# pacificclimate/VIC

Hardware: AMD Instinct MI355X
Metric: cell-timesteps/s (higher is better)
Workload: dtype f64

## Files before the change

vic_amd/csrc/vic_hru_io.hpp:

```cpp
#pragma once
#include <cstddef>
#include "vic_step.hpp"

using namespace vic;

struct LaunchMap {
  int nslot = 0, ccount = 0;
  __host__ __device__ int nblocks(int gcount) const {
    if (nslot == 0) return (gcount + 63) / 64;
    const int ncb = (ccount + 63) / 64;
    return (ncb + 7) / 8 * 8 * nslot;
  }
  VIC_DEV int index(int block, int lane, int gcount) const {
    if (nslot == 0) { const int gi = block * 64 + lane; return gi < gcount ? gi : -1; }
    const int q = block >> 3, cb = q / nslot * 8 + (block & 7), cell = cb * 64 + lane;
    return cell < ccount ? (q % nslot) * ccount + cell : -1;
  }
};

struct KArgs {
  Opt o;
  LaunchMap map;
  int ncell, nhru, nveg_rows, write_fluxes;
  const double* veglib;
  const double* cell_params;
  const int* hpi;
  const double* hpd;
  const double* forcing;
  const unsigned char* snowflag;
  const int* fcol;
  int ncol;
  Dmy dmy;
  double* sd;
  int* si;
  double* flux;
  int* hru_err;
  const int* glist;
  int gcount;
  unsigned long long* ctx;
  double* pin;
  double* ts;
  double* pout;
  int* pslot;
  int* hstate;
  int* list;
  int* count;
  int list_cap;
  int* hkey;
  double* pimp;
  int* lastexp;
  int* jl;
  int phase;
  const int* valid;
};

template <int NN>
VIC_DEV void load_state(const KArgs& a, int g, HruWork<NN>& w, bool node_props = true) {
  const int Nn = a.o.Nnode;
  const size_t nh = a.nhru;
  const double* __restrict__ sd = a.sd;
  const int* __restrict__ si = a.si;
#define SD(row) sd[(size_t)(row) * nh + g]
#define SI(row) si[(size_t)(row) * nh + g]
#pragma unroll
  for (int l = 0; l < 3; l++) { w.moist[l] = SD(SD_MOIST0 + l); w.ice[l] = SD(SD_ICE0 + l); w.layer_T[l] = SD(SD_LAYER_T0 + l); w.evap[l] = 0; }
  SoilEnergy& so = w.so; SnowEnergy& se = w.se; Snow& s = w.snow;
  so.snow_flux = SD(SD_SNOW_FLUX); so.grnd_flux = SD(SD_GRND_FLUX); so.deltaH = SD(SD_DELTAH); so.fusion = SD(SD_FUSION);
  so.LongUnderOut = SD(SD_LONGUNDEROUT); se.Tfoliage = SD(SD_TFOLIAGE);
  s.albedo = SD(SD_SNOW_ALBEDO); s.coldcontent = SD(SD_SNOW_COLDCONTENT); s.coverage = SD(SD_SNOW_COVERAGE);
  s.density = SD(SD_SNOW_DENSITY); s.depth = SD(SD_SNOW_DEPTH); s.pack_temp = SD(SD_SNOW_PACK_TEMP);
  s.pack_water = SD(SD_SNOW_PACK_WATER); s.snow_canopy = SD(SD_SNOW_CANOPY); s.surf_temp = SD(SD_SNOW_SURF_TEMP);
  s.surf_water = SD(SD_SNOW_SURF_WATER); s.swq = SD(SD_SNOW_SWQ); s.tmp_int_storage = SD(SD_SNOW_TMP_INT_STORAGE);
  s.store_swq = SD(SD_SNOW_STORE_SWQ); s.store_coverage = SD(SD_SNOW_STORE_COVERAGE); s.swq_slope = SD(SD_SNOW_SWQ_SLOPE);
  s.max_swq = SD(SD_SNOW_MAX_SWQ);
  s.blowing_flux = 0; s.canopy_vapor_flux = 0; s.mass_error = 0; s.melt = 0; s.Qnet = 0; s.surface_flux = 0; s.vapor_flux = 0;
  w.vv.Wdew = SD(SD_WDEW); w.vv.canopyevap = 0; w.vv.throughfall = 0;
  w.Tcanopy = SD(SD_TCANOPY); so.Tsurf = SD(SD_TSURF); se.AlbedoOver = SD(SD_ALBEDO_OVER); so.AlbedoUnder = SD(SD_ALBEDO_UNDER);
  se.canopy_advection = SD(SD_CANOPY_ADVECTION); se.canopy_latent = SD(SD_CANOPY_LATENT);
  se.canopy_latent_sub = SD(SD_CANOPY_LATENT_SUB); se.canopy_sensible = SD(SD_CANOPY_SENSIBLE);
  se.canopy_refreeze = SD(SD_CANOPY_REFREEZE);
// ... 217 lines not shown
```

vic_amd/csrc/vic_kernels.hpp:

```cpp
#pragma once
#include <cstddef>
#include "vic_glacier.hpp"
#include "vic_profile.hpp"
#include "vic_implicit.hpp"
#include "vic_ctx.hpp"
#include "vic_hru_io.hpp"

using namespace vic;

template <int NN, bool GLAC>
VIC_DEV int hru_prologue(const KArgs& a, int g, const HruId& id, const CellView& cv, const VegLib& vl, const Forcing& fc, const Soil3& s3,
                         HruWork<NN>& w, StepConst& C, bool node_props = true) {
  const Opt& o = a.o;
  const size_t nh = a.nhru;
  const int month = a.dmy.month;
  const int veg_idx = id.veg_idx;
  int err = 0;
  C.veg_idx = veg_idx; C.band = id.band; C.is_art_bare = id.is_art_bare ? 1 : 0;
#pragma unroll
  for (int l = 0; l < 3; l++) C.root[l] = (double)(float)a.hpd[(size_t)(HPD_ROOT0 + l) * nh + g];
  if (o.BLOWING) {
    C.sigma_slope = (double)(float)a.hpd[(size_t)HPD_SIGMA_SLOPE * nh + g]; C.lag_one = (double)(float)a.hpd[(size_t)HPD_LAG_ONE * nh + g];
    C.fetch = (double)(float)a.hpd[(size_t)HPD_FETCH * nh + g];
  } else { C.sigma_slope = 0; C.lag_one = 0; C.fetch = 0; }
// ... 115 lines not shown
      const double blow[4] = {C.sigma_slope, C.lag_one, C.fetch, (double)C.is_art_bare};
      ok = surface_fluxes_glac<NN>(o, cv, vl, s3, fc, a.dmy, C.veg_idx, C.band, C.bare_albedo, C.aero_pet, C.Ra, C.U, C.zref, C.z0, C.disp, blow, w, w.gl,
                                   w.so.NetLongUnder, ge, nlu, nsu, sui);
      SoilEnergy& so = w.so; SnowEnergy& se = w.se;
      so.snow_flux = ge.snow_flux; so.grnd_flux = ge.grnd_flux; so.deltaH = 0; so.fusion = 0; so.LongUnderOut = ge.LongUnderOut;
      so.AlbedoUnder = ge.AlbedoUnder; so.advected_sensible = ge.advected_sensible; so.advection = ge.advection;
      so.deltaCC = ge.deltaCC; so.refreeze_energy = ge.refreeze_energy; so.error = ge.error; so.latent = ge.latent;
      so.latent_sub = ge.latent_sub; so.sensible = ge.sensible; so.NetLongUnder = nlu; so.NetShortUnder = nsu; so.NetShortGrnd = 0;
      se.canopy_advection = 0; se.canopy_latent = 0; se.canopy_latent_sub = 0; se.canopy_sensible = 0; se.canopy_refreeze = 0;
      w.AlbedoOver_avg = 0; w.LongOverIn_avg = 0; w.NetLongOver_avg = 0; w.NetShortOver_avg = 0; w.ShortOverIn_avg = 0;
      w.ShortUnderIn_avg = sui;
      w.deltaCC_glac = ge.deltaCC_glac; w.glacier_flux = ge.glacier_flux; w.glacier_melt_energy = ge.glacier_melt_energy;
      if (!isnan(w.gl.cum_mass_balance) && !isnan(w.gl.mass_balance)) w.gl.cum_mass_balance += w.gl.mass_balance;
    } else {
      ok = surface_fluxes<NN>(o, cv, vl, s3, fc, a.dmy, C, w);
    }
    if (!ok) err |= VICGPU_CELLERR_SOLVER;
  }
  hru_epilogue<NN>(a, g, cv, s3, C, w, err, GLAC);
  PROF_ADD(0, t_kernel);
  PROF_WAVE(0);
  PROF_LANE(1);
}

template <int NN, bool FIRST, bool MULTI>
__global__ __launch_bounds__(64) VIC_WAVES_PER_EU(1, 1) void vic_fd_stage(const KArgs a) {
  const int gi = a.map.index(blockIdx.x, threadIdx.x, a.gcount);
  if (gi < 0) return;
  const int g = a.glist ? a.glist[gi] : gi;
  const Opt& o = a.o;
  const HruId id = hru_id(a, g);
  if (id.run && id.is_glacier) return;
  if (FIRST && a.valid && a.valid[id.c] != CELL_VALID) { a.hstate[g] = 0; return; }
  if (FIRST && !id.run) { store_zero_record(a, g); a.hstate[g] = 0; return; }
  if (!FIRST && (a.hstate[g] & HS_STATE) != 2) return;
  CellView cv{a.cell_params, a.ncell, id.c, o.Nnode, o.Nband};
  VegLib vl{a.veglib};
  Forcing fc{a.forcing, a.snowflag, a.ncell, id.c, o.NR + 1, a.fcol[g], a.ncol};
  const Soil3 s3 = load_soil3(cv);
  const int Nn = node_count<NN>(o.Nnode);
  const CtxRef cx = CtxRef::at(a.ctx, ctx_words<NN>(), g);
  HruWork<NN> w;
  StepConst C;
  SubLoop L;
  int err = 0;
  bool more;
  PROF_T0(t_stage);
  if constexpr (FIRST) {
    err = hru_prologue<NN, false>(a, g, id, cv, vl, fc, s3, w, C, false);
    PROF_ADD(1, t_stage);
    more = !(err & VICGPU_CELLERR_AERO);
    if (more) sf_begin<NN>(o, fc, C, w, L);
  } else {
    SubStep P;
    SurfEB eb;
    SurfSolve sv;
    ctx_get_words(cx, CO_SV, sv, (int)CW_SV_ITER, (int)CW_SV);
    ctx_get(cx, CO_EBM, static_cast<SurfEBMut&>(eb));
    ctx_get_words(cx, CO_EBC, static_cast<SurfEBConst&>(eb), 0, EBC_W_POST);
    surf_cell_fill(eb, cv, vl, s3, fc, eb.hidx, id.veg_idx, a.dmy.month);
    ctx_get(cx, CO_P, P);
    ctx_get_words(cx, CO_L, L, 0, (int)CW_L_HEAD);
    if (MULTI && L.N_steps > 0) ctx_get_words(cx, CO_L, L, (int)CW_L_HEAD, (int)CW_L);
    else zero_substep_sums(L);
    load_untouched_state<NN>(a, g, w);
    if constexpr (MULTI) {
      ctx_get(cx, CO_C, C);
// ... 77 lines not shown
          }
        if constexpr (NN >= NBUCKET / 2) nfrozen = (nfrozen < NBUCKET / 2 - 1) ? nfrozen : NBUCKET / 2 - 1;
        key = nfrozen + (kink ? NBUCKET / 2 : 0);
        a.hkey[g] = key;
      }
      profile_item_store<NN>(o, cv, s3, w.nd, eb.delta_t, eb.frozen_on != 0, a.pin + (size_t)g * Nn * PREC);
      if (o.IMPLICIT) {
        double* __restrict__ im = a.pimp + (size_t)g * Nn * PIMP;
#pragma unroll
        for (int n = 0; n < NN; n++)
          if (n < Nn) {
            im[n * PIMP + PI_MOIST] = w.nd.moist[n]; im[n * PIMP + PI_ICE] = (n == 0) ? eb.delta_t : w.nd.ice[n];
            im[n * PIMP + PI_KAPPA] = w.nd.kappa[n]; im[n * PIMP + PI_CS] = w.nd.Cs[n];
          }
        a.lastexp[g] = -1;
      }
      a.ts[g] = sv.x;
      a.pslot[g] = 0;
      if (o.QUICK_SOLVE) {
        int tmpNnodes = 0;
#pragma unroll
        for (int n = NN - 1; n >= 0; n--)
          if (n <= Nn - 5 && w.nd.T[n] >= 0 && w.nd.T[(n + 1 < NN) ? n + 1 : n] < 0) tmpNnodes = n + 1;
        if (tmpNnodes == 0) tmpNnodes = (w.nd.T[0] <= 0 && w.nd.T[1] >= 0) ? Nn : 3;
        else tmpNnodes += 4;
        a.jl[g] = (sv.stage == SurfSolve::ROOT_QUICK) ? tmpNnodes - 1 : (o.NOFLUX ? Nn : Nn - 1);
      }
      a.pout[(size_t)g * pout_hru_stride(Nn) + pout_key(Nn, 0)] = NAN;
      a.pout[(size_t)g * pout_hru_stride(Nn) + pout_key(Nn, 1)] = NAN;
      a.hstate[g] = 1 | (cls << HS_CLS_SHIFT);
      pend = true;
      PROF_ADD(14, t_put);
    }
  } else {
    PROF_T0(t_end);
    if (more && !sf_end<NN>(o, cv, s3, C, w, L)) err |= VICGPU_CELLERR_SOLVER;
    PROF_ADD(15, t_end);
    hru_epilogue<NN>(a, g, cv, s3, C, w, err, false);
    a.hstate[g] = 0;
  }
  list_append(a.list, a.count, a.list_cap, pend, key, g);
  PROF_ADD(0, t_stage);
  PROF_WAVE(0);
  PROF_LANE(1);
}

struct EArgs {
  Opt o;
  LaunchMap map;
  int ncell, nhru, Nn;
  const int* glist;
  int gcount;
  const double* cell_params;
  const int* hpi;
  unsigned long long* ctx;
  size_t ctx_words;
  double* pout;
  int* pslot;
  double* ts;
  int* jl;
  int* hstate;
  int* list_next;
  int* count_next;
  int list_cap;
  const int* hkey;
  int* profile_next;
  int* pend_list_next;
  int* pend_count_next;
  int pend_cap;
  int list_thr;
  const int* pend_list_cur;
  const int* pend_prefix;
  const int* npend_cur;
  int implicit;
  const double* veglib;
  const double* forcing;
  const int* fcol;
// ... 114 lines not shown
```

vic_amd/csrc/vic_pipeline.hpp:

```cpp
#pragma once
#include <hip/hip_runtime.h>
#include <stdio.h>
#include <stdlib.h>
#include <string.h>
#include <algorithm>
#include <chrono>
#include <condition_variable>
#include <memory>
#include <mutex>
#include <string>
#include <vector>
#include "vicgpu.h"
#include "vic_profile.hpp"
#include "vic_putdata.hpp"
#include "vic_host.hpp"
#include "vic_implicit.hpp"
#include "vic_ctx.hpp"
#include "vic_hru_io.hpp"
#include "vic_kernels.hpp"
#include "vic_aux_kernels.hpp"
#include "vic_records.hpp"
#include "vic_copy_cells.hpp"
#include "vic_params.hpp"
#include "vic_state_update.hpp"
#include "vic_mix_cells.hpp"

using namespace vic;

#define HIPIGN(call) do { hipError_t ign_ = (call); (void)ign_; } while (0)
#define HIPCHK(ctx, call)                                                                              \
  do {                                                                                                 \
    hipError_t e_ = (call);                                                                            \
    if (e_ != hipSuccess) {                                                                            \
      (ctx)->err = std::string(#call) + ": " + hipGetErrorString(e_);                                  \
      return VICGPU_ERR_HIP;                                                                           \
    }                                                                                                  \
  } while (0)

constexpr int RB_LAG = 3, RB_DEPTH = RB_LAG + 1;
struct FdChunk {
  int c0 = 0, ccount = 0;
  DevBuf<int> d_glist;
  int gcount = 0;
  LaunchMap map;
  DevBuf<int> d_list[2];
  DevBuf<int> d_fb_list, d_fb_count;
  DevBuf<int> d_count;
  DevBuf<int> d_plist[2];
  int list_cap = 0;
  int pend_cap = 0;
  PinnedBuf<int> h_count;
  Stream stream;
  Event done, readback[RB_DEPTH];
  std::string err;
  int status = 0;
  long long rounds = 0, steps = 0;
};

struct Domain {
  int ncell = 0, nhru = 0;
  bool domain_ready = false;
  bool any_glacier = false;
  DevBuf<double> d_cp, d_hpd, d_sd, d_flux, d_cell_out, d_accum;
  DevBuf<int> d_hpi, d_si, d_cell_off, d_cell_list, d_hru_err, d_cell_err;
  DevBuf<int> d_valid;
  bool valid_live = false;
  int ncol = 0;
  std::vector<int> cell_col;
  DevBuf<int> d_cell_col;
  DevBuf<int> d_hru_fcol;
  std::vector<int> cell_off, cell_list, copy_key;
  std::vector<int> cell_class;
  MixPlan mix_plan;
  bool fd = false;
  DevBuf<unsigned long long> d_ctx;
  DevBuf<double> d_pin, d_ts, d_pout;
  DevBuf<int> d_hstate, d_pslot, d_hkey, d_lastexp, d_jl;
  DevBuf<double> d_pimp;
  std::vector<FdChunk> chunks;
  bool put_on = false;
  int out_nrow = 0;
  OutLayout out_lay;
  DevBuf<double> d_out_data, d_out_agg, d_pb;
  DevBuf<unsigned char> d_rowagg;
};

constexpr int COPY_NKEY = 4;
constexpr int COPY_KEY_ROWS[COPY_NKEY] = {HPI_BAND, HPI_VEG_CLASS, HPI_IS_GLACIER, HPI_IS_ARTIFICIAL_BARE};

struct Tuning {
  bool node_newton = false;
  int eval_list_pct = 75;
  int nchunk = 1;
  int profile_waves_pct = 100;
  bool xcd_map = true;
  bool trace_rounds = false;
  bool trace = false;
  bool stats = false;
  int copy_stage_mb = 256;
};
static Tuning read_tuning(int node_solver, int ncell) {
  Tuning t;
  t.node_newton = node_solver == VIC_NODE_SOLVER_NEWTON;
  if (const char* ev = getenv("VICGPU_NODE_SOLVER")) t.node_newton = (strcmp(ev, "newton") == 0);
  if (const char* ev = getenv("VICGPU_EVAL_LIST_PCT")) {
    const int pct = atoi(ev);
    if (pct >= 0 && pct <= 100) t.eval_list_pct = pct;
  }
  t.nchunk = (ncell >= 20000) ? 2 : 1;
  if (const char* ev = getenv("VICGPU_CHUNKS")) t.nchunk = atoi(ev);
  if (t.nchunk < 1) t.nchunk = 1;
  if (t.nchunk > 16) t.nchunk = 16;
  if (t.nchunk > ncell) t.nchunk = ncell;
  t.profile_waves_pct = t.nchunk > 1 ? 50 : 100;
  if (const char* ev = getenv("VICGPU_PROFILE_WAVES_PCT")) {
    const int pct = atoi(ev);
    if (pct >= 5 && pct <= 100) t.profile_waves_pct = pct;
  }
  t.xcd_map = getenv("VICGPU_NO_XCD_MAP") == nullptr;
  t.trace_rounds = getenv("VICGPU_TRACE_ROUNDS") != nullptr;
  t.trace = getenv("VICGPU_TRACE") != nullptr;
  t.stats = getenv("VICGPU_STATS") != nullptr;
  if (const char* ev = getenv("VICGPU_COPY_STAGE_MB")) {
    const int mb = atoi(ev);
    if (mb >= 0 && mb <= 65536) t.copy_stage_mb = mb;
  }
  return t;
}


struct RecordsJoin {
  std::mutex m;
  std::condition_variable cv;
  std::vector<int> arrived;
  int queued = 0;
  int status = 0;
  std::string err;
  void start(int nrecords) { arrived.assign(nrecords, 0); queued = 0; status = 0; err.clear(); }
  bool arrive(int k, int nlane) { std::lock_guard<std::mutex> lk(m); return ++arrived[k] == nlane; }
  void join_queued(int k) { { std::lock_guard<std::mutex> lk(m); queued = k + 1; } cv.notify_all(); }
  int wait_queued(int k, std::string* why) {
    std::unique_lock<std::mutex> lk(m);
    cv.wait(lk, [&]() { return queued > k || status != 0; });
    if (status != 0) *why = err;
    return status;
  }
  void fail(int st, const std::string& why) {
    { std::lock_guard<std::mutex> lk(m); if (status == 0) { status = st; err = why; } }
    cv.notify_all();
  }
};

struct Records {
  int nrow = 0, depth = 0;
  DevBuf<int> d_sel_pos;
// ... 46 lines not shown
    std::vector<int> dmy;
    int nsteps = 0;
    Event uploaded;
    Event released;
    bool upload_pending = false, was_current = false;
    Event derive_t0, derive_t1;
    bool derive_timed = false;
  } slot[2];
  int cur = -1, staged = -1;
  Stream stream, copy_stream;
  Records rec;
  std::vector<Event> ev;
  int ev_used = 0;
  int write_fluxes = 1;
  int steps_done = 0;
  int profile_waves = 0;
  int ev_steps = 0;
  int out_step_ratio = 1;
  int retire_mask = 0;
};

struct PertLists {
  int nsrc;
  const int* col_src;
  int src_base;
  int ngroup;
  const int* col_group;
  int group_base;
  const double* pert;
};

static int* valid_table(const vicgpu_ctx* c) { return c->dom.valid_live ? c->dom.d_valid.get() : nullptr; }

static hipStream_t records_stream(const vicgpu_ctx* c) { return c->rec.dl ? (hipStream_t)c->rec.dl : (hipStream_t)c->stream; }

static void records_report_reduce(vicgpu_ctx* c) {
  Records& R = c->rec;
  float ms = 0;
  if (R.reduce_timed && hipEventElapsedTime(&ms, R.reduce_t0, R.reduce_t1) == hipSuccess)
    fprintf(stderr, "[vicgpu] records reduce: %d groups, %d members, a %s per group, %d rows: %.4f ms\n", R.ngroup, R.nnz,
            R.lane_per_group ? "lane" : "wave", R.nrow, ms);
  R.reduce_timed = false;
}

static void free_records(vicgpu_ctx* c) {
  if (c->rec.depth > 0) HIPIGN(hipStreamSynchronize(records_stream(c)));
  records_report_reduce(c);
  c->rec = Records();
}

static void drop_forcing(vicgpu_ctx* c) {
  c->chunk_steps = 0;
  c->dmy.clear();
  c->cur = c->staged = -1;
  c->d_forcing = nullptr; c->d_snowflag = nullptr;
}

static void free_domain(vicgpu_ctx* c) {
  free_records(c);
  c->dom = Domain();
  drop_forcing(c);
}

static const int* forcing_col_row(const Domain& d) { return d.d_hru_fcol ? d.d_hru_fcol.get() : d.d_hpi.get() + (size_t)HPI_CELL * d.nhru; }

template <int NN>
static hipError_t launch_hru(const KArgs& ka, hipStream_t st, bool ordinary, bool glacier) {
  const int nblk = ka.map.nblocks(ka.gcount);
  if constexpr (NN == 3) {
    if (ordinary) hipLaunchKernelGGL((vic_hru_step<NN, false>), dim3(nblk), dim3(64), 0, st, ka);
  }
  if (glacier) hipLaunchKernelGGL((vic_hru_step<NN, true>), dim3(nblk), dim3(64), 0, st, ka);
  return hipGetLastError();
}

template <int NN>
static hipError_t launch_fd_stage(const KArgs& ka, bool multi, hipStream_t st) {
  const dim3 grid(ka.map.nblocks(ka.gcount)), block(64);
  if (ka.phase == 0) {
    if (multi) hipLaunchKernelGGL((vic_fd_stage<NN, true, true>), grid, block, 0, st, ka);
    else hipLaunchKernelGGL((vic_fd_stage<NN, true, false>), grid, block, 0, st, ka);
  } else {
    if (multi) hipLaunchKernelGGL((vic_fd_stage<NN, false, true>), grid, block, 0, st, ka);
    else hipLaunchKernelGGL((vic_fd_stage<NN, false, false>), grid, block, 0, st, ka);
  }
  return hipGetLastError();
}

using ProfileKernel = void (*)(const PArgs);
template <int NN>
constexpr ProfileKernel profile_kernel(bool newton) {
  if constexpr (NN == 10) return newton ? vic_profile_solve_reg<NN, true> : vic_profile_solve_reg<NN, false>;
  else return newton ? vic_profile_solve_lockstep<NN, true> : vic_profile_solve_lockstep<NN, false>;
}

template <int NN>
static hipError_t launch_profile(const PArgs& pa, int nmax, int resident_waves, bool newton, hipStream_t st) {
  int nblk = (nmax + 63) / 64;
  if (nblk > resident_waves) nblk = resident_waves;
  if (nblk < 1) nblk = 1;
  hipLaunchKernelGGL(profile_kernel<NN>(newton), dim3(nblk), dim3(64), 0, st, pa);
  return hipGetLastError();
}

template <int NN>
static int profile_resident_waves(int device, bool newton) {
  int per_cu = 0, ncu = 0;
  const hipError_t e = hipOccupancyMaxActiveBlocksPerMultiprocessor(&per_cu, profile_kernel<NN>(newton), 64, 0);
  if (e != hipSuccess || per_cu <= 0) per_cu = 8;
  if (hipDeviceGetAttribute(&ncu, hipDeviceAttributeMultiprocessorCount, device) != hipSuccess || ncu <= 0) ncu = 256;
  return per_cu * ncu;
}

constexpr int CNT_LIST_STRIDE = 64, CNT_CURSOR = 128, CNT_NPEND = 160, CNT_PREFIX = 192, CNT_STRIPES = 288,
              CNT_STRIPES_STRIDE = PEND_STRIPES * PEND_CNT_STRIDE, CNT_TOTAL = CNT_STRIPES + 2 * CNT_STRIPES_STRIDE;
static_assert(NBUCKET <= CNT_LIST_STRIDE && CNT_PREFIX + PEND_STRIPES + 1 <= CNT_STRIPES && CNT_STRIPES % 32 == 0, "counter block layout");
static inline int* cnt_list(int* d_count, int l) { return d_count + l * CNT_LIST_STRIDE; }
static inline int* cnt_stripes(int* d_count, int l) { return d_count + CNT_STRIPES + l * CNT_STRIPES_STRIDE; }
static inline int cnt_pending(const int* h_count, int l) {
  int n = 0;
  for (int s = 0; s < PEND_STRIPES; s++) n += h_count[CNT_STRIPES + l * CNT_STRIPES_STRIDE + s * PEND_CNT_STRIDE];
  return n;
}

static int fd_read_count(FdChunk* ch, int which, int* nsolve, int* npending) {
  HIPCHK(ch, hipMemcpyAsync(ch->h_count, ch->d_count, sizeof(int) * CNT_TOTAL, hipMemcpyDeviceToHost, ch->stream));
  HIPCHK(ch, hipStreamSynchronize(ch->stream));
  int n = 0;
  for (int b = 0; b < NBUCKET; b++) n += ch->h_count[which * CNT_LIST_STRIDE + b];
  *nsolve = n;
  *npending = cnt_pending(ch->h_count, which);
  return VICGPU_OK;
}

#define NODE_DISPATCH(Nnode, F, ...)                                                                                          \
  (node_bound(Nnode) == 10 ? F<10>(__VA_ARGS__)                                                                           \
                           : node_bound(Nnode) == VIC_MID_NODES ? F<VIC_MID_NODES>(__VA_ARGS__) : F<VIC_MAX_NODES>(__VA_ARGS__))

static KArgs make_kargs(const vicgpu_ctx* c) {
  const Domain& d = c->dom;
  KArgs ka{};
  ka.o = c->o; ka.ncell = d.ncell; ka.nhru = d.nhru; ka.gcount = d.nhru; ka.nveg_rows = c->nveg_rows;
  ka.write_fluxes = (c->write_fluxes || d.put_on) ? 1 : 0;
  ka.veglib = c->d_veglib; ka.cell_params = d.d_cp; ka.hpi = d.d_hpi; ka.hpd = d.d_hpd; ka.sd = d.d_sd; ka.si = d.d_si; ka.flux = d.d_flux;
  ka.hru_err = d.d_hru_err; ka.ctx = d.d_ctx; ka.pin = d.d_pin; ka.ts = d.d_ts; ka.pout = d.d_pout; ka.pslot = d.d_pslot;
  ka.hstate = d.d_hstate; ka.hkey = d.d_hkey; ka.pimp = d.d_pimp; ka.lastexp = d.d_lastexp; ka.jl = d.d_jl;
  ka.valid = valid_table(c);
  ka.fcol = forcing_col_row(d); ka.ncol = d.ncol;
// ... 8 lines not shown
  ca.valid = valid_table(c); ca.retire_mask = c->retire_mask;
  return ca;
}
static PArgs profile_args(const vicgpu_ctx* c, const FdChunk* ch) {
  const Domain& d = c->dom;
  PArgs pa{};
  pa.pin = d.d_pin; pa.ts = d.d_ts; pa.pout = d.d_pout; pa.pslot = d.d_pslot; pa.jl = d.d_jl; pa.cap = ch->list_cap;
  pa.Nn = c->o.Nnode; pa.NOFLUX = c->o.NOFLUX; pa.EXP_TRANS = c->o.EXP_TRANS; pa.TFALLBACK = c->o.TFALLBACK;
  pa.next = ch->d_count + CNT_CURSOR; pa.pend_prefix = ch->d_count + CNT_PREFIX; pa.pend_out = ch->d_count + CNT_NPEND;
  return pa;
}
static EArgs eval_args(const vicgpu_ctx* c, const FdChunk* ch, const KArgs& ka) {
  const Domain& d = c->dom;
  EArgs ea{};
  ea.o = c->o; ea.ncell = d.ncell; ea.nhru = d.nhru; ea.Nn = c->o.Nnode; ea.glist = ch->d_glist; ea.gcount = ch->gcount; ea.map = ch->map;
  ea.cell_params = d.d_cp; ea.hpi = d.d_hpi; ea.ctx = d.d_ctx; ea.ctx_words = NODE_DISPATCH(c->o.Nnode, ctx_words);
  ea.pout = d.d_pout; ea.pslot = d.d_pslot; ea.ts = d.d_ts; ea.jl = d.d_jl; ea.hstate = d.d_hstate; ea.hkey = d.d_hkey;
  ea.list_cap = ch->list_cap; ea.pend_cap = ch->pend_cap; ea.profile_next = ch->d_count + CNT_CURSOR;
  ea.pend_prefix = ch->d_count + CNT_PREFIX; ea.npend_cur = ch->d_count + CNT_NPEND; ea.implicit = c->o.IMPLICIT;
  ea.veglib = c->d_veglib; ea.forcing = ka.forcing; ea.fcol = ka.fcol; ea.ncol = ka.ncol; ea.month = ka.dmy.month;
  return ea;
}
static IArgs implicit_args(const vicgpu_ctx* c, const FdChunk* ch) {
  const Domain& d = c->dom;
  IArgs ia{};
  ia.ncell = d.ncell; ia.nhru = d.nhru; ia.Nband = c->o.Nband; ia.pimp = d.d_pimp; ia.hpi = d.d_hpi; ia.cell_params = d.d_cp;
  ia.hkey = d.d_hkey; ia.lastexp = d.d_lastexp; ia.fb_list = ch->d_fb_list; ia.fb_count = ch->d_fb_count; ia.cursor = ch->d_fb_count + NBUCKET;
  return ia;
}

static int fd_step(vicgpu_ctx* c, FdChunk* ch, KArgs ka) {
  const int Nn = c->o.Nnode;
  hipStream_t st = ch->stream;
  if (c->dom.any_glacier) HIPCHK(ch, NODE_DISPATCH(Nn, launch_hru, ka, st, false, true));
  HIPCHK(ch, hipMemsetAsync(ch->d_count, 0, sizeof(int) * CNT_TOTAL, st));
  int cur = 0;
  ka.phase = 0; ka.list = ch->d_list[cur]; ka.count = cnt_list(ch->d_count, cur); ka.list_cap = ch->list_cap;
  HIPCHK(ch, NODE_DISPATCH(Nn, launch_fd_stage, ka, c->o.NF > 1, st));
  PArgs pa = profile_args(c, ch);
  EArgs ea = eval_args(c, ch, ka);
  const IArgs ia = c->o.IMPLICIT ? implicit_args(c, ch) : IArgs{};
  const int list_thr = (int)((long long)ch->gcount * c->tune.eval_list_pct / 100);
  const int FREE_ROUNDS = 6;
  const int nsub = c->o.NF;
  for (int p = 1; p <= nsub; p++) {
    int nmax = ch->gcount;
    int npend = -1;
    int rb_list[RB_DEPTH];
    int rb_first = -1;
    for (int round = 0;; round++) {
      pa.list = ch->d_list[cur]; pa.count = cnt_list(ch->d_count, cur); pa.count_zero = cnt_list(ch->d_count, cur ^ 1);
      pa.pend_counts = cnt_list(ch->d_count, cur); pa.pend_stripes = cnt_stripes(ch->d_count, cur);
      pa.pend_stripes_zero = cnt_stripes(ch->d_count, cur ^ 1);
      if (c->o.IMPLICIT) {
        HIPCHK(ch, hipMemsetAsync(ch->d_fb_count, 0, sizeof(int) * (NBUCKET + 1), st));
        const int nblk = std::min(std::max((nmax + 63) / 64, 1), 4096);
        hipLaunchKernelGGL(vic_profile_solve_implicit, dim3(nblk), dim3(64), 0, st, pa, ia);
        HIPCHK(ch, hipGetLastError());
        pa.list = ch->d_fb_list; pa.count = ch->d_fb_count;
      }
      HIPCHK(ch, NODE_DISPATCH(Nn, launch_profile, pa, nmax, c->profile_waves, c->tune.node_newton, st));
      ea.list_next = ch->d_list[cur ^ 1]; ea.count_next = cnt_list(ch->d_count, cur ^ 1);
      ea.pend_list_next = ch->d_plist[cur ^ 1]; ea.pend_count_next = cnt_stripes(ch->d_count, cur ^ 1);
      ea.pend_list_cur = ch->d_plist[cur];
      ea.list_thr = round > 0 ? list_thr : -1;
      const bool sparse = npend >= 0 && npend <= ea.list_thr;
      hipLaunchKernelGGL(vic_surf_eval, dim3(sparse ? ((npend + 63) / 64 > 0 ? (npend + 63) / 64 : 1) : ea.map.nblocks(ch->gcount)), dim3(64), 0, st, ea);
      HIPCHK(ch, hipGetLastError());
      cur ^= 1;
      ch->rounds++;
      if (c->tune.trace_rounds) {
        int n = 0, np = 0;
        if (fd_read_count(ch, cur, &n, &np) != VICGPU_OK) return VICGPU_ERR_HIP;
        fprintf(stderr, "vicgpu rounds: chunk %d sub-step %d round %d leaves %d solves + %d evaluation-only of %d\n", (int)(ch - &c->dom.chunks[0]), p, round, n, np - n, ch->gcount);
      }
      if (round + 2 >= FREE_ROUNDS) {
        const int slot = round % RB_DEPTH;
        if (rb_first < 0) rb_first = round;
        HIPCHK(ch, hipMemcpyAsync(ch->h_count + slot * CNT_TOTAL, ch->d_count, sizeof(int) * CNT_TOTAL, hipMemcpyDeviceToHost, st));
        HIPCHK(ch, hipEventRecord(ch->readback[slot], st));
        rb_list[slot] = cur;
      }
      if (rb_first >= 0 && round - RB_LAG >= rb_first) {
        const int slot = (round - RB_LAG) % RB_DEPTH;
        HIPCHK(ch, hipEventSynchronize(ch->readback[slot]));
        const int* h = ch->h_count + slot * CNT_TOTAL;
        int n = 0;
        for (int b = 0; b < NBUCKET; b++) n += h[rb_list[slot] * CNT_LIST_STRIDE + b];
        const int np = cnt_pending(h, rb_list[slot]);
        if (np == 0) break;
        nmax = n;
        npend = np;
      }
    }
    ka.phase = p; ka.list = ch->d_list[cur]; ka.count = cnt_list(ch->d_count, cur);
    HIPCHK(ch, NODE_DISPATCH(Nn, launch_fd_stage, ka, c->o.NF > 1, st));
    if (p < nsub) {
      int n = 0, ne = 0;
      const int r = fd_read_count(ch, cur, &n, &ne);
      if (r != VICGPU_OK) return r;
      if (n == 0) break;
    }
  }
  ch->steps++;
  return VICGPU_OK;
}

static hipError_t launch_put_data(const vicgpu_ctx* c, hipStream_t st, int c0, int ccount, int s) {
  OArgs a;
  a.o = c->o; a.lay = c->dom.out_lay; a.ncell = c->dom.ncell; a.nhru = c->dom.nhru; a.c0 = c0; a.ccount = ccount;
  a.rec = s < 0 ? -1 : 0; a.out_step_ratio = c->out_step_ratio;
  a.cell_off = c->dom.d_cell_off; a.cell_list = c->dom.d_cell_list; a.cell_params = c->dom.d_cp; a.veglib = c->d_veglib;
  a.hpi = c->dom.d_hpi; a.hpd = c->dom.d_hpd; a.sd = c->dom.d_sd; a.si = c->dom.d_si; a.flux = c->dom.d_flux;
  a.forcing = s < 0 ? nullptr : c->d_forcing + (size_t)s * VIC_NFORCE * (c->o.NR + 1) * c->dom.ncol;
  a.cell_col = c->dom.d_cell_col; a.ncol = c->dom.ncol;
  a.cell_out = c->dom.d_cell_out; a.out_data = c->dom.d_out_data; a.out_agg = c->dom.d_out_agg; a.pb = c->dom.d_pb;
  a.valid = valid_table(c);
  const unsigned nblk = (unsigned)((ccount + 63) / 64);
  hipLaunchKernelGGL(vic_put_zero, dim3(nblk, (c->dom.out_nrow + PUT_AGG_ROWS - 1) / PUT_AGG_ROWS), dim3(64), 0, st, a);
  if (c->o.Nnode > VIC_MID_NODES) hipLaunchKernelGGL(vic_put_sum_deep, dim3(nblk, PUT_NPART), dim3(64), 0, st, a);
  else hipLaunchKernelGGL(vic_put_sum, dim3(nblk, PUT_NPART), dim3(64), 0, st, a);
  hipLaunchKernelGGL(vic_put_finish, dim3(nblk), dim3(64), 0, st, a);
  if (s >= 0)
    hipLaunchKernelGGL(vic_put_aggregate, dim3(nblk, (c->dom.out_nrow + PUT_AGG_ROWS - 1) / PUT_AGG_ROWS), dim3(64), 0, st, a, c->dom.d_rowagg);
  return hipGetLastError();
}
// ... 58 lines not shown
  if (!groups) {
    float* dst = R.out + (size_t)k * R.nrow * ld + c0;
    const float* src = R.slot[s].d_out + c0;
    if ((size_t)ccount == nc && ld == nc) e = hipMemcpyAsync(dst, src, sizeof(float) * nc * R.nrow, hipMemcpyDeviceToHost, dl);
    else e = hipMemcpy2DAsync(dst, sizeof(float) * ld, src, sizeof(float) * nc, sizeof(float) * ccount, R.nrow, hipMemcpyDeviceToHost, dl);
    if (e != hipSuccess) return failed(e);
  }
  if (R.err) e = hipMemcpyAsync(R.err + (size_t)k * ld + c0, R.slot[s].d_err + c0, sizeof(int) * ccount, hipMemcpyDeviceToHost, dl);
  if (e != hipSuccess) return failed(e);
  if (!groups) e = hipEventRecord(R.landed[(size_t)lane * R.last_nrecords + k], dl);
  else if (R.join->arrive(k, R.nlane)) {
    if ((e = records_join(c, k)) == hipSuccess) R.join->join_queued(k);
  }
  return e == hipSuccess ? VICGPU_OK : failed(e);
}

static void set_step_inputs(const vicgpu_ctx* c, KArgs& ka, int s) {
  const size_t nsub = c->o.NR + 1;
  ka.forcing = c->d_forcing + (size_t)s * VIC_NFORCE * nsub * c->dom.ncol;
  ka.snowflag = c->d_snowflag + (size_t)s * nsub * c->dom.ncell;
  const int* d = &c->dmy[(size_t)s * VIC_NDMY];
  ka.dmy.month = d[VIC_DMY_MONTH]; ka.dmy.day_in_year = d[VIC_DMY_DAY_IN_YEAR]; ka.dmy.hour = d[VIC_DMY_HOUR];
  ka.dmy.day = d[VIC_DMY_DAY]; ka.dmy.year = d[VIC_DMY_YEAR];
}

static int fd_chunk_steps(const StepPlan& plan, FdChunk* ch) {
  vicgpu_ctx* c = plan.c;
  HIPCHK(ch, hipSetDevice(c->device));
  KArgs ka = plan.ka;
  CArgs ca = plan.ca;
  ka.glist = ch->d_glist; ka.gcount = ch->gcount; ka.map = ch->map;
  ca.c0 = ch->c0; ca.ccount = ch->ccount;
  const int lane = (int)(ch - &c->dom.chunks[0]);
  for (int s = plan.step0; s < plan.step0 + plan.nsteps; s++) {
    if (plan.records && lane == 0 && s == plan.step0 + plan.nsteps - plan.ratio && s > plan.step0) HIPCHK(ch, hipEventRecord(c->ev[0], ch->stream));
    set_step_inputs(c, ka, s);
    const long long r0 = ch->rounds;
    const auto t0 = std::chrono::steady_clock::now();
    const int r = fd_step(c, ch, ka);
    if (r != VICGPU_OK) return r;
    if (c->tune.trace) {
      HIPCHK(ch, hipStreamSynchronize(ch->stream));
      fprintf(stderr, "[vicgpu] step %d hour %d: %.2f ms, %lld rounds\n", s, ka.dmy.hour,
              std::chrono::duration<double, std::milli>(std::chrono::steady_clock::now() - t0).count(), ch->rounds - r0);
    }
    hipLaunchKernelGGL(vic_cell_reduce, dim3((ch->ccount + 255) / 256), dim3(256), 0, ch->stream, ca);
    HIPCHK(ch, hipGetLastError());
    if (c->dom.put_on) HIPCHK(ch, launch_put_data(c, ch->stream, ch->c0, ch->ccount, s));
    if (plan.records && (s - plan.step0 + 1) % plan.ratio == 0) {
      const int re = records_emit(c, &ch->err, lane, ch->stream, ch->c0, ch->ccount, (s - plan.step0) / plan.ratio);
      if (re != VICGPU_OK) return re;
    }
  }
  HIPCHK(ch, hipEventRecord(ch->done, ch->stream));
  return VICGPU_OK;
}

static int fd_chunk_run(const StepPlan& plan, FdChunk* ch) {
  const int r = fd_chunk_steps(plan, ch);
  Records& R = plan.c->rec;
  if (r != VICGPU_OK && plan.records && R.ngroup > 0) R.join->fail(r, ch->err);
  return r;
}


static int domain_tables(vicgpu_ctx* c, const double* cell_params, const int* hpi, const double* hpd, const int* cell_hru_offset,
                         const int* cell_hru_list) {
  Domain& d = c->dom;
  hipStream_t st = c->stream;
  const size_t ncell = d.ncell, nhru = d.nhru;
  const int Nn = c->opt.Nnode, Nb = c->opt.Nband;
  for (size_t g = 0; g < nhru; g++) if (hpi[HPI_IS_GLACIER * nhru + g]) d.any_glacier = true;
  HIPCHK(c, d.d_cp.alloc(VIC_CPX_NROW(Nn, Nb) * ncell));
  HIPCHK(c, d.d_cp.upload(st, cell_params, 0, VICGPU_CP_NROW(Nn, Nb) * ncell));
  hipLaunchKernelGGL(vic_derive_cell_params, dim3((c->dom.ncell + 255) / 256), dim3(256), 0, st, c->dom.d_cp, c->dom.ncell, Nn, Nb);
  HIPCHK(c, hipGetLastError());
  HIPCHK(c, d.d_hpi.alloc(HPI_NROW * nhru));
  HIPCHK(c, d.d_hpi.upload(st, hpi));
  HIPCHK(c, d.d_hpd.alloc(HPD_NROW * nhru));
  HIPCHK(c, d.d_hpd.upload(st, hpd));
  HIPCHK(c, d.d_cell_off.alloc(ncell + 1));
  HIPCHK(c, d.d_cell_off.upload(st, cell_hru_offset));
  HIPCHK(c, d.d_cell_list.alloc(nhru));
  HIPCHK(c, d.d_cell_list.upload(st, cell_hru_list));
  d.cell_off.assign(cell_hru_offset, cell_hru_offset + ncell + 1);
// ... 47 lines not shown
    ch.c0 = (int)((long long)ncell * k / nchunk);
    ch.ccount = (int)((long long)ncell * (k + 1) / nchunk) - ch.c0;
    std::vector<int> gl(cell_hru_list + cell_hru_offset[ch.c0], cell_hru_list + cell_hru_offset[ch.c0 + ch.ccount]);
    std::sort(gl.begin(), gl.end());
    ch.gcount = (int)gl.size();
    ch.map = LaunchMap();
    if (ch.ccount > 0 && ch.gcount % ch.ccount == 0 && c->tune.xcd_map) {
      const int nslot = ch.gcount / ch.ccount;
      bool regular = true;
      for (int sl = 0; sl < nslot && regular; sl++)
        for (int i = 0; i < ch.ccount; i++)
          if (gl[(size_t)sl * ch.ccount + i] != sl * ncell + ch.c0 + i || hpi[(size_t)HPI_CELL * nhru + gl[(size_t)sl * ch.ccount + i]] != ch.c0 + i) {
            regular = false;
            break;
          }
      if (regular) { ch.map.nslot = nslot; ch.map.ccount = ch.ccount; }
    }
    const size_t gn = ch.gcount > 0 ? ch.gcount : 1;
    ch.list_cap = (int)gn;
    HIPCHK(c, ch.d_glist.alloc(gn));
    if (ch.gcount) HIPCHK(c, ch.d_glist.upload(c->stream, gl.data()));
    HIPCHK(c, ch.d_list[0].alloc(gn * NBUCKET));
    HIPCHK(c, ch.d_list[1].alloc(gn * NBUCKET));
    HIPCHK(c, ch.d_count.alloc(CNT_TOTAL));
    ch.pend_cap = 64 * ((ch.map.nblocks(ch.gcount) + PEND_STRIPES - 1) / PEND_STRIPES);
    if (ch.pend_cap < 64) ch.pend_cap = 64;
    HIPCHK(c, ch.d_plist[0].alloc((size_t)ch.pend_cap * PEND_STRIPES));
    HIPCHK(c, ch.d_plist[1].alloc((size_t)ch.pend_cap * PEND_STRIPES));
    if (c->o.IMPLICIT) {
      HIPCHK(c, ch.d_fb_list.alloc(gn * NBUCKET));
      HIPCHK(c, ch.d_fb_count.alloc(NBUCKET + 1));
    }
    HIPCHK(c, ch.h_count.alloc((size_t)CNT_TOTAL * RB_DEPTH));
    HIPCHK(c, ch.stream.create());
    HIPCHK(c, ch.done.create(hipEventDisableTiming));
    for (Event& e : ch.readback) HIPCHK(c, e.create(hipEventDisableTiming));
  }
  return VICGPU_OK;
}

constexpr int COPY_NTABLE = 4;
template <typename F>
static hipError_t copy_table(vicgpu_ctx* c, int t, int what, F&& f) {
  Domain& d = c->dom;
  const int Nn = c->opt.Nnode;
  const bool state = (what & VICGPU_COPY_STATE) != 0, balance = (what & VICGPU_COPY_BALANCE) != 0;
  switch (t) {
    case 0: return state ? f(d.d_sd.get(), (int)VICGPU_SD_NROW(Nn), (size_t)d.nhru, false) : hipSuccess;
    case 1: return state ? f(d.d_si.get(), (int)VICGPU_SI_NROW(Nn), (size_t)d.nhru, false) : hipSuccess;
    case 2: return state ? f(d.d_flux.get(), (int)FX_NROW, (size_t)d.nhru, false) : hipSuccess;
    default: return balance ? f(d.d_pb.get(), (int)PBX_NROW, (size_t)d.ncell, true) : hipSuccess;
  }
}

static std::string copy_fault_text(const CopyPlan& p) {
  const char* rule = p.fault == COPY_CELL_RANGE ? "a cell is outside the domain"
                     : p.fault == COPY_DST_REPEATS ? "the destination repeats"
                                                   : copy_pair_fault_text(p.fault);
  return "copy_cells: pair " + std::to_string(p.index) + ": " + rule;
}

template <typename T>
static int d2h(vicgpu_ctx* c, T* dst, const DevBuf<T>& src, size_t count) {
  if (!c || !dst || !src) return VICGPU_ERR_ARG;
  HIPCHK(c, hipSetDevice(c->device));
  HIPCHK(c, hipStreamSynchronize(c->stream));
  HIPCHK(c, src.download(c->stream, dst, 0, count));
  return VICGPU_OK;
}
// ... 12 lines not shown
```

vic_amd/csrc/vicgpu_api.hip:

```cpp
#include <hip/hip_runtime.h>
#include <stdio.h>
#include <stdlib.h>
#include <string.h>
#include <algorithm>
#include <cmath>
#include <memory>
#include <string>
#include <thread>
#include <vector>
#include "vicgpu.h"
#include "vic_glacier.hpp"
#include "vic_profile.hpp"
#include "vic_putdata.hpp"
#include "vic_host.hpp"
#include "vic_checks.hpp"
#include "vic_implicit.hpp"
#include "vic_ctx.hpp"
#include "vic_hru_io.hpp"
#include "vic_kernels.hpp"
#include "vic_aux_kernels.hpp"
#include "vic_records.hpp"
#include "vic_copy_cells.hpp"
#include "vic_params.hpp"
#include "vic_state_update.hpp"
// ... 388 lines not shown
      HIPCHK(c, hipEventRecord(c->ev[2 * i], c->stream));
      HIPCHK(c, launch_hru<3>(ka, c->stream, true, c->dom.any_glacier));
      HIPCHK(c, hipEventRecord(c->ev[2 * i + 1], c->stream));
      hipLaunchKernelGGL(vic_cell_reduce, dim3((c->dom.ncell + 255) / 256), dim3(256), 0, c->stream, ca);
      HIPCHK(c, hipGetLastError());
      if (c->dom.put_on) HIPCHK(c, launch_put_data(c, c->stream, 0, c->dom.ncell, s));
      c->steps_done++;
      if (records && i == per - 1) {
        const int re = records_emit(c, &c->err, 0, c->stream, 0, c->dom.ncell, (s - step0) / per);
        if (re != VICGPU_OK) return re;
      }
    }
    c->ev_used = per;
    c->ev_steps = per;
    return VICGPU_OK;
  }
  HIPCHK(c, hipEventRecord(c->ev[0], c->stream));
  for (FdChunk& ch : c->dom.chunks) {
    HIPCHK(c, hipStreamWaitEvent(ch.stream, c->ev[0], 0));
    ch.status = VICGPU_OK;
    ch.err.clear();
  }
  if (c->dom.chunks.size() == 1) c->dom.chunks[0].status = fd_chunk_run(plan, &c->dom.chunks[0]);
  else {
    std::vector<std::thread> th;
    for (FdChunk& ch : c->dom.chunks) th.emplace_back([&plan, &ch]() { ch.status = fd_chunk_run(plan, &ch); });
    for (std::thread& t : th) t.join();
  }
  int status = VICGPU_OK;
  for (FdChunk& ch : c->dom.chunks) {
    if (ch.status != VICGPU_OK && status == VICGPU_OK) { status = ch.status; c->err = ch.err; }
  }
  if (status != VICGPU_OK) {
    for (FdChunk& ch : c->dom.chunks) HIPIGN(hipStreamSynchronize(ch.stream));
    return status;
  }
  for (FdChunk& ch : c->dom.chunks) HIPCHK(c, hipStreamWaitEvent(c->stream, ch.done, 0));
  HIPCHK(c, hipEventRecord(c->ev[1], c->stream));
  c->ev_used = 1;
  c->ev_steps = per;
  c->steps_done += nsteps;
  return VICGPU_OK;
}

int vicgpu_step(vicgpu_ctx* c, int step0, int nsteps) {
  if (!c) return VICGPU_ERR_ARG;
  if (!c->dom.domain_ready || !c->d_veglib || !c->d_forcing || c->chunk_steps <= 0) return VICGPU_ERR_STATE;
  if (step0 < 0 || nsteps <= 0 || step0 + nsteps > c->chunk_steps) return VICGPU_ERR_ARG;
  HIPCHK(c, hipSetDevice(c->device));
  return step_impl(c, step0, nsteps, 0);
}

int vicgpu_synchronize(vicgpu_ctx* c) {
  if (!c) return VICGPU_ERR_ARG;
  HIPCHK(c, hipSetDevice(c->device));
  HIPCHK(c, hipStreamSynchronize(c->stream));
  if (c->rec.dl) HIPCHK(c, hipStreamSynchronize(c->rec.dl));
  return VICGPU_OK;
}

int vicgpu_last_kernel_ms(vicgpu_ctx* c, double* ms_per_launch, int* nlaunch) {
  if (!c || !ms_per_launch) return VICGPU_ERR_ARG;
  HIPCHK(c, hipSetDevice(c->device));
  HIPCHK(c, hipStreamSynchronize(c->stream));
  double tot = 0;
  for (int i = 0; i < c->ev_used; i++) {
    float ms = 0;
// ... 725 lines not shown
  if (step0 < 0 || nrecords < 1 || (long long)step0 + (long long)nrecords * ratio > c->chunk_steps || ld < c->dom.ncell) return VICGPU_ERR_ARG;
  HIPCHK(c, hipSetDevice(c->device));
  if (!out || !is_pinned(out) || (cell_err && !is_pinned(cell_err))) return VICGPU_ERR_ARG;
  Records& R = c->rec;
  if (R.ngroup > 0 && ld != c->dom.ncell) return VICGPU_ERR_STATE;
  const size_t nev = (size_t)R.nlane * nrecords;
  if (R.landed.size() < nev) {
    const size_t had = R.landed.size();
    R.landed.resize(nev);
    for (size_t i = had; i < nev; i++) HIPCHK(c, R.landed[i].create(hipEventDisableTiming));
  }
  if (R.ngroup > 0) {
    if (R.reduced.size() < (size_t)nrecords) {
      const size_t had = R.reduced.size();
      R.reduced.resize(nrecords);
      for (size_t i = had; i < (size_t)nrecords; i++) HIPCHK(c, R.reduced[i].create(hipEventDisableTiming));
    }
    if (c->tune.stats && !R.reduce_t0) {
      HIPCHK(c, R.reduce_t0.create());
      HIPCHK(c, R.reduce_t1.create());
    }
    R.join->start(nrecords);
  }
  R.follows = R.last_nrecords > 0;
  R.out = out; R.err = cell_err; R.ld = ld;
  R.last_nrecords = nrecords;
  int r = step_impl(c, step0, nrecords * ratio, ratio);
  if (r == VICGPU_OK) {
    const hipError_t e = hipEventRecord(R.drained, records_stream(c));
    if (e != hipSuccess) { c->err = std::string("hipEventRecord: ") + hipGetErrorString(e); r = VICGPU_ERR_HIP; }
  }
  if (r != VICGPU_OK) {
    HIPIGN(hipStreamSynchronize(c->stream));
    for (FdChunk& ch : c->dom.chunks) HIPIGN(hipStreamSynchronize(ch.stream));
    HIPIGN(hipStreamSynchronize(records_stream(c)));
    R.last_nrecords = 0;
  }
  return r;
}
int vicgpu_run_records(vicgpu_ctx* c, int step0, int nrecords, float* out, int* cell_err) {
  return c ? run_records_impl(c, step0, nrecords, out, cell_err, c->dom.ncell) : VICGPU_ERR_ARG;
}

int vicgpu_records_wait(vicgpu_ctx* c, int k) {
  if (!c) return VICGPU_ERR_ARG;
  const Records& R = c->rec;
  if (R.depth < 1 || R.last_nrecords < 1) return VICGPU_ERR_STATE;
  if (k < -1 || k >= R.last_nrecords) return VICGPU_ERR_ARG;
  HIPCHK(c, hipSetDevice(c->device));
  if (k < 0) { HIPCHK(c, hipEventSynchronize(R.drained)); return VICGPU_OK; }
  if (R.ngroup > 0) { HIPCHK(c, hipEventSynchronize(R.reduced[k])); return VICGPU_OK; }
  for (int lane = 0; lane < R.nlane; lane++) HIPCHK(c, hipEventSynchronize(R.landed[(size_t)lane * R.last_nrecords + k]));
  return VICGPU_OK;
}

}
```

Measured before the change: 4.165 million.

## Defer early-finishing HRUs and glacier pass past first readback; add optional tail stream

```diff
diff --git a/vic_amd/csrc/vic_hru_io.hpp b/vic_amd/csrc/vic_hru_io.hpp
--- a/vic_amd/csrc/vic_hru_io.hpp
+++ b/vic_amd/csrc/vic_hru_io.hpp
@@ -46,6 +46,8 @@
   int* list;
   int* count;
   int list_cap;
+  int* early_list;
+  int* early_count;
   int* hkey;
   double* pimp;
   int* lastexp;
diff --git a/vic_amd/csrc/vic_kernels.hpp b/vic_amd/csrc/vic_kernels.hpp
--- a/vic_amd/csrc/vic_kernels.hpp
+++ b/vic_amd/csrc/vic_kernels.hpp
@@ -171,7 +171,11 @@
   const HruId id = hru_id(a, g);
   if (id.run && id.is_glacier) return;
   if (FIRST && a.valid && a.valid[id.c] != CELL_VALID) { a.hstate[g] = 0; return; }
-  if (FIRST && !id.run) { store_zero_record(a, g); a.hstate[g] = 0; return; }
+  if (FIRST && !id.run) { a.hstate[g] = 0; return; }
+  if (!FIRST && !id.run) {
+    if (a.phase == 1 && !(a.valid && a.valid[id.c] != CELL_VALID)) store_zero_record(a, g);
+    return;
+  }
   if (!FIRST && (a.hstate[g] & HS_STATE) != 2) return;
   CellView cv{a.cell_params, a.ncell, id.c, o.Nnode, o.Nband};
   VegLib vl{a.veglib};
@@ -315,6 +319,10 @@
       pend = true;
       PROF_ADD(14, t_put);
     }
+  } else if constexpr (FIRST) {
+    const int k = atomicAdd(a.early_count, 1);
+    if (k < a.list_cap) a.early_list[k] = g;
+    a.hstate[g] = 0;
   } else {
     PROF_T0(t_end);
     if (more && !sf_end<NN>(o, cv, s3, C, w, L)) err |= VICGPU_CELLERR_SOLVER;
@@ -326,6 +334,28 @@
   PROF_ADD(0, t_stage);
   PROF_WAVE(0);
   PROF_LANE(1);
+}
+
+template <int NN>
+__global__ __launch_bounds__(64) void vic_fd_early(const KArgs a) {
+  const Opt& o = a.o;
+  const int n = *a.early_count < a.list_cap ? *a.early_count : a.list_cap;
+  for (int i = blockIdx.x * 64 + threadIdx.x; i < n; i += gridDim.x * 64) {
+    const int g = a.early_list[i];
+    const HruId id = hru_id(a, g);
+    CellView cv{a.cell_params, a.ncell, id.c, o.Nnode, o.Nband};
+    VegLib vl{a.veglib};
+    Forcing fc{a.forcing, a.snowflag, a.ncell, id.c, o.NR + 1, a.fcol[g], a.ncol};
+    const Soil3 s3 = load_soil3(cv);
+    HruWork<NN> w;
+    StepConst C;
+    SubLoop L;
+    int err = hru_prologue<NN, false>(a, g, id, cv, vl, fc, s3, w, C, false);
+    const bool more = !(err & VICGPU_CELLERR_AERO);
+    if (more) sf_begin<NN>(o, fc, C, w, L);
+    if (more && !sf_end<NN>(o, cv, s3, C, w, L)) err |= VICGPU_CELLERR_SOLVER;
+    hru_epilogue<NN>(a, g, cv, s3, C, w, err, false);
+  }
 }
 
 struct EArgs {
diff --git a/vic_amd/csrc/vic_pipeline.hpp b/vic_amd/csrc/vic_pipeline.hpp
--- a/vic_amd/csrc/vic_pipeline.hpp
+++ b/vic_amd/csrc/vic_pipeline.hpp
@@ -50,7 +50,12 @@
   int list_cap = 0;
   int pend_cap = 0;
   PinnedBuf<int> h_count;
+  DevBuf<int> d_early;
   Stream stream;
+  Stream tail_own;
+  Event tail_ready;
+  Event tail_done;
+  bool tail_pending = false;
   Event done, readback[RB_DEPTH];
   std::string err;
   int status = 0;
@@ -97,6 +102,7 @@
   bool trace_rounds = false;
   bool trace = false;
   bool stats = false;
+  bool tail_stream = false;
   int copy_stage_mb = 256;
 };
 static Tuning read_tuning(int node_solver, int ncell) {
@@ -121,6 +127,7 @@
   t.trace_rounds = getenv("VICGPU_TRACE_ROUNDS") != nullptr;
   t.trace = getenv("VICGPU_TRACE") != nullptr;
   t.stats = getenv("VICGPU_STATS") != nullptr;
+  if (const char* ev = getenv("VICGPU_TAIL_STREAM")) t.tail_stream = atoi(ev) == 1;
   if (const char* ev = getenv("VICGPU_COPY_STAGE_MB")) {
     const int mb = atoi(ev);
     if (mb >= 0 && mb <= 65536) t.copy_stage_mb = mb;
@@ -233,6 +240,8 @@
 
 static int* valid_table(const vicgpu_ctx* c) { return c->dom.valid_live ? c->dom.d_valid.get() : nullptr; }
 
+static hipStream_t chunk_tail(const vicgpu_ctx* c, const FdChunk& ch) { return c->tune.tail_stream ? (hipStream_t)ch.tail_own : (hipStream_t)ch.stream; }
+
 static hipStream_t records_stream(const vicgpu_ctx* c) { return c->rec.dl ? (hipStream_t)c->rec.dl : (hipStream_t)c->stream; }
 
 static void records_report_reduce(vicgpu_ctx* c) {
@@ -288,6 +297,12 @@
   return hipGetLastError();
 }
 
+template <int NN>
+static hipError_t launch_fd_early(const KArgs& ka, int n, hipStream_t st) {
+  hipLaunchKernelGGL((vic_fd_early<NN>), dim3(std::min(std::max((n + 63) / 64, 1), 4096)), dim3(64), 0, st, ka);
+  return hipGetLastError();
+}
+
 using ProfileKernel = void (*)(const PArgs);
 template <int NN>
 constexpr ProfileKernel profile_kernel(bool newton) {
@@ -314,7 +329,8 @@
 }
 
 constexpr int CNT_LIST_STRIDE = 64, CNT_CURSOR = 128, CNT_NPEND = 160, CNT_PREFIX = 192, CNT_STRIPES = 288,
-              CNT_STRIPES_STRIDE = PEND_STRIPES * PEND_CNT_STRIDE, CNT_TOTAL = CNT_STRIPES + 2 * CNT_STRIPES_STRIDE;
+              CNT_STRIPES_STRIDE = PEND_STRIPES * PEND_CNT_STRIDE, CNT_EARLY = CNT_STRIPES + 2 * CNT_STRIPES_STRIDE,
+              CNT_TOTAL = CNT_EARLY + 32;
 static_assert(NBUCKET <= CNT_LIST_STRIDE && CNT_PREFIX + PEND_STRIPES + 1 <= CNT_STRIPES && CNT_STRIPES % 32 == 0, "counter block layout");
 static inline int* cnt_list(int* d_count, int l) { return d_count + l * CNT_LIST_STRIDE; }
 static inline int* cnt_stripes(int* d_count, int l) { return d_count + CNT_STRIPES + l * CNT_STRIPES_STRIDE; }
@@ -389,10 +405,10 @@
 static int fd_step(vicgpu_ctx* c, FdChunk* ch, KArgs ka) {
   const int Nn = c->o.Nnode;
   hipStream_t st = ch->stream;
-  if (c->dom.any_glacier) HIPCHK(ch, NODE_DISPATCH(Nn, launch_hru, ka, st, false, true));
   HIPCHK(ch, hipMemsetAsync(ch->d_count, 0, sizeof(int) * CNT_TOTAL, st));
   int cur = 0;
   ka.phase = 0; ka.list = ch->d_list[cur]; ka.count = cnt_list(ch->d_count, cur); ka.list_cap = ch->list_cap;
+  ka.early_list = ch->d_early; ka.early_count = ch->d_count + CNT_EARLY;
   HIPCHK(ch, NODE_DISPATCH(Nn, launch_fd_stage, ka, c->o.NF > 1, st));
   PArgs pa = profile_args(c, ch);
   EArgs ea = eval_args(c, ch, ka);
@@ -400,6 +416,7 @@
   const int list_thr = (int)((long long)ch->gcount * c->tune.eval_list_pct / 100);
   const int FREE_ROUNDS = 6;
   const int nsub = c->o.NF;
+  int n_early = -1;
   for (int p = 1; p <= nsub; p++) {
     int nmax = ch->gcount;
     int npend = -1;
@@ -445,10 +462,19 @@
         int n = 0;
         for (int b = 0; b < NBUCKET; b++) n += h[rb_list[slot] * CNT_LIST_STRIDE + b];
         const int np = cnt_pending(h, rb_list[slot]);
+        n_early = h[CNT_EARLY];
         if (np == 0) break;
         nmax = n;
         npend = np;
       }
+    }
+    if (p == 1) {
+      if (ch->tail_pending) {
+        HIPCHK(ch, hipStreamWaitEvent(st, ch->tail_done, 0));
+        ch->tail_pending = false;
+      }
+      if (c->dom.any_glacier) HIPCHK(ch, NODE_DISPATCH(Nn, launch_hru, ka, st, false, true));
+      if (n_early != 0) HIPCHK(ch, NODE_DISPATCH(Nn, launch_fd_early, ka, n_early < 0 ? ch->gcount : n_early, st));
     }
     ka.phase = p; ka.list = ch->d_list[cur]; ka.count = cnt_list(ch->d_count, cur);
     HIPCHK(ch, NODE_DISPATCH(Nn, launch_fd_stage, ka, c->o.NF > 1, st));
@@ -573,6 +599,7 @@
   ka.glist = ch->d_glist; ka.gcount = ch->gcount; ka.map = ch->map;
   ca.c0 = ch->c0; ca.ccount = ch->ccount;
   const int lane = (int)(ch - &c->dom.chunks[0]);
+  const hipStream_t tail = chunk_tail(c, *ch);
   for (int s = plan.step0; s < plan.step0 + plan.nsteps; s++) {
     if (plan.records && lane == 0 && s == plan.step0 + plan.nsteps - plan.ratio && s > plan.step0) HIPCHK(ch, hipEventRecord(c->ev[0], ch->stream));
     set_step_inputs(c, ka, s);
@@ -587,11 +614,25 @@
     }
     hipLaunchKernelGGL(vic_cell_reduce, dim3((ch->ccount + 255) / 256), dim3(256), 0, ch->stream, ca);
     HIPCHK(ch, hipGetLastError());
-    if (c->dom.put_on) HIPCHK(ch, launch_put_data(c, ch->stream, ch->c0, ch->ccount, s));
-    if (plan.records && (s - plan.step0 + 1) % plan.ratio == 0) {
-      const int re = records_emit(c, &ch->err, lane, ch->stream, ch->c0, ch->ccount, (s - plan.step0) / plan.ratio);
+    const bool record_end = plan.records && (s - plan.step0 + 1) % plan.ratio == 0;
+    const bool split = tail != (hipStream_t)ch->stream && (c->dom.put_on || record_end);
+    if (split) {
+      HIPCHK(ch, hipEventRecord(ch->tail_ready, ch->stream));
+      HIPCHK(ch, hipStreamWaitEvent(tail, ch->tail_ready, 0));
+    }
+    if (c->dom.put_on) HIPCHK(ch, launch_put_data(c, tail, ch->c0, ch->ccount, s));
+    if (record_end) {
+      const int re = records_emit(c, &ch->err, lane, tail, ch->c0, ch->ccount, (s - plan.step0) / plan.ratio);
       if (re != VICGPU_OK) return re;
     }
+    if (split) {
+      HIPCHK(ch, hipEventRecord(ch->tail_done, tail));
+      ch->tail_pending = true;
+    }
+  }
+  if (ch->tail_pending) {
+    HIPCHK(ch, hipStreamWaitEvent(ch->stream, ch->tail_done, 0));
+    ch->tail_pending = false;
   }
   HIPCHK(ch, hipEventRecord(ch->done, ch->stream));
   return VICGPU_OK;
@@ -705,9 +746,15 @@
       HIPCHK(c, ch.d_fb_count.alloc(NBUCKET + 1));
     }
     HIPCHK(c, ch.h_count.alloc((size_t)CNT_TOTAL * RB_DEPTH));
+    HIPCHK(c, ch.d_early.alloc(gn));
     HIPCHK(c, ch.stream.create());
     HIPCHK(c, ch.done.create(hipEventDisableTiming));
     for (Event& e : ch.readback) HIPCHK(c, e.create(hipEventDisableTiming));
+  }
+  for (FdChunk& ch : d.chunks) {
+    if (c->tune.tail_stream) HIPCHK(c, ch.tail_own.create());
+    HIPCHK(c, ch.tail_ready.create(hipEventDisableTiming));
+    HIPCHK(c, ch.tail_done.create(hipEventDisableTiming));
   }
   return VICGPU_OK;
 }
diff --git a/vic_amd/csrc/vicgpu_api.hip b/vic_amd/csrc/vicgpu_api.hip
--- a/vic_amd/csrc/vicgpu_api.hip
+++ b/vic_amd/csrc/vicgpu_api.hip
@@ -444,7 +444,7 @@
     if (ch.status != VICGPU_OK && status == VICGPU_OK) { status = ch.status; c->err = ch.err; }
   }
   if (status != VICGPU_OK) {
-    for (FdChunk& ch : c->dom.chunks) HIPIGN(hipStreamSynchronize(ch.stream));
+    for (FdChunk& ch : c->dom.chunks) { HIPIGN(hipStreamSynchronize(ch.stream)); HIPIGN(hipStreamSynchronize(chunk_tail(c, ch))); }
     return status;
   }
   for (FdChunk& ch : c->dom.chunks) HIPCHK(c, hipStreamWaitEvent(c->stream, ch.done, 0));
@@ -1236,7 +1236,7 @@
   }
   if (r != VICGPU_OK) {
     HIPIGN(hipStreamSynchronize(c->stream));
-    for (FdChunk& ch : c->dom.chunks) HIPIGN(hipStreamSynchronize(ch.stream));
+    for (FdChunk& ch : c->dom.chunks) { HIPIGN(hipStreamSynchronize(ch.stream)); HIPIGN(hipStreamSynchronize(chunk_tail(c, ch))); }
     HIPIGN(hipStreamSynchronize(records_stream(c)));
     R.last_nrecords = 0;
   }
```

Result: no change. 4.152 million (-0.3%).
